# sharckhai/drsa-audio

Measured on AMD Instinct MI355X. Metric: explained samples/sec (LRP+DRSA k=4), higher is better.
Workload: dtype fp32; 1 GPU; GTZAN-128 HeatmapGenerator: LRP (WSquare/Gamma/Epsilon name map) + DRSA subspace heatmaps, K=4 at layer j=7 (conv3 block, d=64), sorted info dict; global_batch=512, per_gpu_batch=512, input=128x128 log-mel, parallelism=data-parallel x1 (no collective on the data path), launch=single process, one_device_rehearsal=False

## Files before the change

### drsa_audio_amd/csrc/conv_bwd_b.hip

```cpp
#include "lrp_conv_kernel.h"

#ifndef DRSA_CONV_CIC_BWD32
#define DRSA_CONV_CIC_BWD32 8
#endif
#ifndef DRSA_CONV_CIC_BWD64_32
#define DRSA_CONV_CIC_BWD64_32 8
#endif

CONV_TABLE(kTableBwdB,
    BWD_SET(64, 32, DRSA_CONV_CIC_BWD64_32),
    BWD_SET(32, 32, DRSA_CONV_CIC_BWD32))

#ifdef DRSA_CONV_STAMP
extern "C" int drsa_amd_debug_conv_stamps(void* buf) {
  return (int)hipMemcpyToSymbol(HIP_SYMBOL(drsa_conv::g_conv_stamps), &buf, sizeof(buf));
}
#endif
```

### drsa_audio_amd/csrc/lrp_conv.h

```cpp
#pragma once
#include <stdint.h>

enum XMode { XM_NONE = 0, XM_MUL = 1, XM_SPLIT = 2 };
enum PostMode { POST_NONE = 0, POST_DIV = 1, POST_MASK = 2, POST_DIV_RING = 3 };

struct ConvArgs {
  const float* in;
  const uint8_t* in_amax;
  const float* wts;
  const float* bias;
  const float* den_map;
  const float* den_const4;
  const float* x;
  const float* den;
  float* out;
  uint8_t* out_amax;
  float* out_den;
  int H, W;
  int cin, cout;
  int clones;
  int xmode, post;
  float eps;
  int den_ring_only;
  int den_shared;
};

#include <hip/hip_runtime.h>
int drsa_first_conv_pool(const ConvArgs& a, int cout_p, int ng, int B, hipStream_t s);
```

### drsa_audio_amd/csrc/lrp_conv.hip

```cpp
#include "common.h"
#include "lrp_conv.h"
#include "lrp_conv_kernel.h"

#include <stdlib.h>

#define DRSA_CONV_TABLES(X) \
  X(FwdA) X(FwdB) X(FwdC) X(FwdD) X(FwdE) X(BwdA) X(BwdB) X(BwdC) X(FwdBfA) X(FwdBfB) X(FwdBfC) X(FwdP4) X(BwdBfA) X(BwdBfB)

namespace drsa_conv {
#define DRSA_CONV_DECLARE(T) extern const Table kTable##T;
DRSA_CONV_TABLES(DRSA_CONV_DECLARE)
extern const Table kTableSmall;
}

namespace {
using drsa_conv::Entry;
using namespace drsa_conv;

#define DRSA_CONV_ADDRESS(T) &drsa_conv::kTable##T,
const drsa_conv::Table* kTables[] = {DRSA_CONV_TABLES(DRSA_CONV_ADDRESS)};

int pad32(int c) { return (c + 31) / 32 * 32; }

#ifndef DRSA_CONV_FWD128_TW
#define DRSA_CONV_FWD128_TW 8
#endif
const Entry* find(int cin_p, int cout_p, int W, int ng, int amode, int epi, int et = 0, int pw = 2) {
  int th = 8, tw, mw;
  const bool fwd_t16 = epi != EPI_BWD && et == 0 && cout_p == 64;
  const bool bwd_t16 = epi == EPI_BWD && et == 0 && ((cout_p == 64 && cin_p <= 128) || cout_p == 128);
  if (W >= 32 && epi != EPI_BWD && et == 0 && cout_p == 128 && DRSA_CONV_FWD128_TW != 32) {
    tw = DRSA_CONV_FWD128_TW;
    mw = tw == 8 ? 4 : 8;
  } else if (W >= 32 && (fwd_t16 || bwd_t16)) { tw = 16; mw = 8; }
  else if (W >= 32) { tw = 32; mw = 8; }
  else { tw = 8; mw = 4; }
  for (const drsa_conv::Table* t : kTables)
    for (int i = 0; i < t->n; ++i) {
      const Entry& e = t->entries[i];
      if (e.cin_p == cin_p && e.cout_p == cout_p && e.th == th && e.tw == tw && e.mw == mw && e.ng == ng &&
          e.amode == amode && e.epi == epi && e.et == et && e.pw == pw)
        return &e;
    }
  return nullptr;
}

#ifndef DRSA_CONV_SMALL_WG
#define DRSA_CONV_SMALL_WG 512
#endif
const Entry* small_tile(const Entry* e, int H, int W, int batch) {
  if (e->th != 8 || e->tw != 8) return e;
  if ((int64_t)((H + 7) / 8) * ((W + 7) / 8) * batch >= DRSA_CONV_SMALL_WG) return e;
  for (int i = 0; i < drsa_conv::kTableSmall.n; ++i) {
    const Entry& c = drsa_conv::kTableSmall.entries[i];
    if (c.cin_p == e->cin_p && c.cout_p == e->cout_p && c.ng == e->ng && c.amode == e->amode && c.epi == e->epi &&
        c.et == e->et && c.pw == e->pw)
      return &c;
  }
  return e;
}

int launch(const Entry* e0, const ConvArgs& args, int batch, hipStream_t s) {
  DRSA_REQUIRE((int64_t)(args.cin > args.cout ? args.cin : args.cout) * args.H * args.W < ((int64_t)1 << 31),
               "conv: one sample's channels x H x W must stay below 2^31");
  const Entry* e = small_tile(e0, args.H, args.W, batch);
  DRSA_SMEM(e->fn, e->lds);
  const int tiles = ((args.H + e->th - 1) / e->th) * ((args.W + e->tw - 1) / e->tw);
  hipLaunchKernelGGL(e->fn, dim3(tiles, batch), dim3(kThreads), e->lds, s, args);
  DRSA_LAUNCH_CHECK();
  return DRSA_OK;
}

int cin_pad(int cin) { return cin == 1 ? 1 : pad32(cin); }

const Entry* find_fwd(int cin, int cout, int W, int ng, int pool, int bf16) {
  return find(bf16 ? pad32(cin) : cin_pad(cin), pad32(cout), W, ng, A_DENSE, pool ? EPI_FWD_POOL : EPI_FWD_RELU,
              bf16 ? 1 : 0, pool == 2 ? 4 : 2);
}

const Entry* find_bwd(int cin, int cout, int W, int ng, int sparse, int bf16, int pool_w) {
  return find(pad32(cin), pad32(cout), W, ng, sparse ? A_POOLSPARSE : A_DENSE, EPI_BWD, bf16 ? 1 : 0, pool_w);
}

// ... 76 lines not shown
  return launch(e, a, c.Bq, (hipStream_t)stream);
}

}

extern "C" {

size_t drsa_amd_conv_weight_floats(int cin, int cout, int ng) {
  return (size_t)ng * 9 * cin_pad(cin) * pad32(cout);
}

size_t drsa_amd_conv_weight_bf16_elems(int cin, int cout, int ng) {
  return (size_t)ng * 9 * pad32(cin) * pad32(cout);
}

int drsa_amd_conv_fwd_has_kernel(int cin, int cout, int W, int ng, int pool, int bf16) {
  if (cin == 1 && !bf16 && pool == 1) return 1;
  if (pool < 0 || pool > 2 || ng < 1 || ng > 3 || (bf16 && cin == 1)) return 0;
  return find_fwd(cin, cout, W, ng, pool, bf16) != nullptr;
}

int drsa_amd_conv_bwd_has_kernel_bf16(int cin, int cout, int W, int ng, int sparse) {
  if (cin < 16 || ng != 1) return 0;
  return find_bwd(cin, cout, W, ng, sparse, 1, 2) != nullptr;
}

int drsa_amd_conv_bwd_has_kernel_pw(int cin, int cout, int W, int ng, int pool_w) {
  if (cin < 2 || (pool_w != 2 && pool_w != 4) || (pool_w == 4 && (W / 4) % 4 != 0)) return 0;
  return find_bwd(cin, cout, W, ng, 1, 0, pool_w) != nullptr;
}
// ... 79 lines not shown
```

### drsa_audio_amd/csrc/lrp_conv_kernel.h

```cpp
#pragma once
#include "common.h"
#include "lrp_conv.h"

#include <type_traits>

#ifndef DRSA_CONV_PD_BWD
#define DRSA_CONV_PD_BWD 2
#endif
#ifndef DRSA_CONV_BWD_ES
#define DRSA_CONV_BWD_ES 1
#endif
#ifndef DRSA_CONV_BWD_WPE
#define DRSA_CONV_BWD_WPE 3
#endif
#ifndef DRSA_CONV_PIN_SMALL
#define DRSA_CONV_PIN_SMALL 1
#endif
#ifndef DRSA_CONV_PD_SMALL
#define DRSA_CONV_PD_SMALL 3
#endif
#ifndef DRSA_CONV_SMALL_WPE
#define DRSA_CONV_SMALL_WPE 4
#endif
#ifndef DRSA_CONV_SMALL_ES
// ... 11 lines not shown
#ifndef DRSA_CONV_FWD_WPE_128
#define DRSA_CONV_FWD_WPE_128 3
#endif
#ifndef DRSA_CONV_FWD_WPE_WIDE
#define DRSA_CONV_FWD_WPE_WIDE 3
#endif
#ifndef DRSA_CONV_FWD_WPE
#define DRSA_CONV_FWD_WPE 3
#endif

namespace drsa_conv {

constexpr int kThreads = 256;

#ifdef DRSA_CONV_STAMP
static __device__ unsigned long long* g_conv_stamps;
#endif

__device__ const float g_zero_bias3[3 * 128] = {};

template <int V, int M>
constexpr int round_up() { return (V + M - 1) / M * M; }

constexpr int halo_stride(int hx, int mw) {
  int r = hx;
  const int want = (mw == 8) ? 16 : 8;
  while (r % 32 != want) ++r;
  return r;
}

enum AMode { A_DENSE = 0, A_POOLSPARSE = 1 };
enum Epi { EPI_FWD_POOL = 0, EPI_FWD_RELU = 1, EPI_BWD = 2 };

constexpr int XO = 3;

constexpr int bf_stride(int hx) {
  int r = hx;
  while (r % 16 != 8) ++r;
  return r;
}

template <int CIN, int COUT, int TH, int TW, int MW, int CIC, int NG, int AMODE, int EPI, int ET = 0, int PW = 2>
struct ConvCfg {
  static constexpr int CIN_ = CIN, COUT_ = COUT, TH_ = TH, TW_ = TW, MW_ = MW, CIC_ = CIC, NG_ = NG;
  static constexpr int AMODE_ = AMODE, EPI_ = EPI;
  static constexpr bool BF = ET == 1;
  static constexpr int HY = TH + 2, HX = TW + 2;
  static constexpr int HXB = bf_stride(HX);
  static constexpr size_t bf_halo_floats = (size_t)2 * HY * HXB * 4;
  static constexpr size_t bf_w_floats = (size_t)NG * 9 * 2 * COUT * 4;
  static constexpr int RS = halo_stride(HX + XO, MW);
  static constexpr int PLANE_RAW = HY * RS;
  static constexpr int PLANE = PLANE_RAW + ((PLANE_RAW % 32) == 0 ? 4 : 0);
  static constexpr int MTW = 2 * MW;
  static constexpr int MTH = 32 / MTW;
  static constexpr int MTX = TW / MTW;
  static constexpr int MT = (TH / MTH) * MTX;
  static constexpr int NT = COUT / 32;
  static constexpr int WM = MT >= 4 ? 4 : MT;
  static constexpr int WN = (4 / WM) < NT ? (4 / WM) : NT;
  static constexpr int MPW = MT / WM;
  static constexpr int NPW = NT / WN;
  static constexpr int KC = 9 * CIC;
  static constexpr int KCP = round_up<KC, 2>();
  static constexpr int NCHUNK = CIN / CIC;
  static constexpr int TWP = (TW == 32) ? 48 : TW;
  static constexpr bool SMALL_BWD = EPI == EPI_BWD && NG == 1 && CIC <= 8 && COUT <= 32;
  static constexpr int ES = (EPI == EPI_BWD && WN == 1) ? (SMALL_BWD ? DRSA_CONV_SMALL_ES : DRSA_CONV_BWD_ES) : 1;
  static constexpr int TCH = WN * 32 / ES;
  static constexpr size_t staging_floats =
      BF ? bf_halo_floats + bf_w_floats : (size_t)CIC * PLANE + (size_t)NG * KCP * COUT;
  static constexpr size_t epi_floats = (size_t)TCH * TH * TWP;
  static constexpr size_t lds_floats = staging_floats > epi_floats ? staging_floats : epi_floats;
  static constexpr int WPE = BF ? (COUT <= 64 ? DRSA_CONV_BF_WPE : 1)
                             : (EPI == EPI_BWD && NG == 1) ? (SMALL_BWD ? DRSA_CONV_SMALL_WPE : DRSA_CONV_BWD_WPE)
                             : (EPI != EPI_BWD && CIC <= 8 && COUT <= 32 && NG <= 2 ? DRSA_CONV_FWD_WPE
                                : EPI != EPI_BWD && CIC <= 8 && NG <= 2 && COUT == 64 ? DRSA_CONV_FWD_WPE_WIDE
                                : EPI != EPI_BWD && CIC <= 4 && NG <= 2 && COUT == 128 && TW == 8 ? DRSA_CONV_FWD_WPE_128 : 1);
  static constexpr bool PIN = SMALL_BWD && DRSA_CONV_PIN_SMALL;
  static constexpr int PD = PIN ? DRSA_CONV_PD_SMALL : DRSA_CONV_PD_BWD > 0 && EPI >= EPI_BWD ? DRSA_CONV_PD_BWD : 1;
  static_assert(TH % MTH == 0 && TW % MTW == 0, "tile must be a multiple of the M-tile");
  static_assert(COUT % 32 == 0, "COUT must be padded to 32");
  static_assert(CIN % CIC == 0, "CIN must be a multiple of the chunk");
  static_assert(MT % WM == 0 && NT % WN == 0 && WM * WN <= 4, "wave split");
  static_assert(!BF || (CIC == 16 && (EPI < EPI_BWD ? AMODE == A_DENSE : EPI == EPI_BWD)),
                "bf16: 16-channel chunks; dense forward, or the per-clone backward (dense or pool-sparse g)");
  static_assert(PW == 2 || (PW == 4 && (EPI == EPI_FWD_POOL || (EPI == EPI_BWD && AMODE == A_POOLSPARSE &&
                                                                  (ET == 1 || TW % 16 == 0)))),
                "2x4 pool windows: the forward pool epilogue, or the backward's pool-sparse staging (fp32: "
                "tiles of whole float4 cell groups)");
  static constexpr int PW_ = PW;
};

template <class Cfg, int NT_ = kThreads>
struct Stager {
  static constexpr int CIN = Cfg::CIN_, COUT = Cfg::COUT_, TH = Cfg::TH_, TW = Cfg::TW_, CIC = Cfg::CIC_;
  static constexpr int NG = Cfg::NG_, HY = Cfg::HY, HX = Cfg::HX, RS = Cfg::RS, PLANE = Cfg::PLANE;
  static constexpr int KC = Cfg::KC, KCP = Cfg::KCP;
  static constexpr bool DENSE = Cfg::AMODE_ == A_DENSE;
  static constexpr int Q4 = TW / 4, DROWS = CIC * HY;
  static constexpr int DI = (DROWS * Q4 + NT_ - 1) / NT_, DH = (DROWS * 2 + NT_ - 1) / NT_;
  static constexpr int CY = TH / 2 + 2, CX = TW / 2 + 2, Q8 = TW / 8 > 0 ? TW / 8 : 1, SROWS = CIC * CY;
  static constexpr int SI = (SROWS * Q8 + NT_ - 1) / NT_, SH = (SROWS * 2 + NT_ - 1) / NT_;
  static constexpr bool P4 = !DENSE && Cfg::PW_ == 4;
  static constexpr int Q16 = TW / 16 > 0 ? TW / 16 : 1;
  static constexpr int SI4 = (SROWS * Q16 + NT_ - 1) / NT_;
  static constexpr int NI = DENSE ? DI : P4 ? SI4 : SI, NH = DENSE ? DH : SH;
  static constexpr int NWV = NG * KCP * (COUT / 4), WIT = (NWV + NT_ - 1) / NT_;
  float4 st_i[NI];
  uint32_t st_ia[DENSE ? 1 : NI];
  float st_h[NH];
  int st_ha[DENSE ? 1 : NH];
  float4 st_w[WIT];

  __device__ __forceinline__ void load(const ConvArgs& a, int c0, int tid, int ty0, int tx0, int bq, int bs) {
    const int H = a.H, W = a.W, H2 = H >> 1, W2 = W >> 1;
    const int W4 = W >> 2;
    const float* __restrict__ inb = a.in + (size_t)bq * a.cin * (DENSE ? H * W : H2 * (P4 ? W4 : W2));
    const uint8_t* __restrict__ amb = DENSE ? nullptr : a.in_amax + (size_t)bs * a.cin * H2 * (P4 ? W4 : W2);
    if constexpr (P4) {
      const int qy0 = (ty0 >> 1) - 1, cx0 = tx0 >> 2;
#pragma unroll
      for (int it = 0; it < SI4; ++it) {
        const int i = tid + it * NT_;
        const int row = i / Q16, q = i % Q16;
        const int ci = row / CY, ry = row % CY;
        const int cy = qy0 + ry, cx = cx0 + 4 * q, c = c0 + ci;
        const bool ok = i < SROWS * Q16 && cy >= 0 && cy < H2 && c < a.cin && cx < W4;
        const int o = ok ? (c * H2 + cy) * W4 + cx : 0;
        const float4 v = *reinterpret_cast<const float4*>(inb + o);
// ... 101 lines not shown
        const int i = tid + it * NT_;
        const int row = i >> 1, side = i & 1;
        const int ci = row / CY, ry = row % CY;
        const int cy = qy0 + ry, cx = side ? qx0 + CX - 1 : qx0, c = c0 + ci;
        const bool ok = i < SROWS * 2 && cy >= 0 && cy < H2 && cx >= 0 && cx < W2 && c < a.cin;
        const int o = ok ? (c * H2 + cy) * W2 + cx : 0;
        const float v = inb[o];
        const int am = (int)amb[o];
        st_h[it] = ok ? v : 0.f;
        st_ha[it] = ok ? am : 4;
      }
    }
#pragma unroll
    for (int it = 0; it < WIT; ++it) {
      const int idx = tid + it * NT_;
      const int g = idx / (KCP * (COUT / 4)), rem = idx % (KCP * (COUT / 4));
      const int k = rem / (COUT / 4), c4 = (rem % (COUT / 4)) * 4;
      const bool ok = idx < NWV && k < KC;
      const float4 v = *reinterpret_cast<const float4*>(a.wts + (ok ? ((size_t)g * 9 * CIN + c0 * 9 + k) * COUT + c4 : 0));
      st_w[it] = ok ? v : make_float4(0.f, 0.f, 0.f, 0.f);
    }
  }

  __device__ __forceinline__ static void put_cell(float* halo, int ci, int ry, int rx, float v, int sb) {
    float* d = halo + ci * PLANE + (2 * ry - 1) * RS + 2 * rx - 1 + XO;
    if (ry > 0) *reinterpret_cast<float2*>(d) = make_float2(sb == 0 ? v : 0.f, sb == 1 ? v : 0.f);
    if (ry < CY - 1) *reinterpret_cast<float2*>(d + RS) = make_float2(sb == 2 ? v : 0.f, sb == 3 ? v : 0.f);
  }

  __device__ __forceinline__ static void put_cell4(float* halo, int ci, int ry, int rx, float v, int sb) {
    float* d = halo + ci * PLANE + (2 * ry - 1) * RS + 4 * rx;
    if (ry > 0)
      *reinterpret_cast<float4*>(d) = make_float4(sb == 0 ? v : 0.f, sb == 1 ? v : 0.f, sb == 2 ? v : 0.f, sb == 3 ? v : 0.f);
    if (ry < CY - 1)
// ... 65 lines not shown
          put_cell(halo, row / CY, row % CY, side ? CX - 1 : 0, st_h[it], st_ha[it]);
        }
      }
    }
#pragma unroll
    for (int it = 0; it < WIT; ++it) {
      const int idx = tid + it * NT_;
      if (idx < NWV) *reinterpret_cast<float4*>(wl + (size_t)idx * 4) = st_w[it];
    }
  }
};

template <class Cfg, int PD = 1>
__device__ __forceinline__ void mfma_chunk(const float* halo, const float* wl, const int (&pix_off)[Cfg::MPW],
                                           int lane, int wn, f32x16 (&acc)[Cfg::NG_][Cfg::MPW][Cfg::NPW]) {
  constexpr int MPW = Cfg::MPW, NPW = Cfg::NPW, NG = Cfg::NG_, COUT = Cfg::COUT_;
  constexpr int KC = Cfg::KC, KCP = Cfg::KCP, PLANE = Cfg::PLANE, RS = Cfg::RS, EPI = Cfg::EPI_;
  const int h = lane >> 5;
  constexpr int DLT[3] = {1, RS - 2, PLANE - 2 * RS - 2};
  int xb[MPW][3];
#pragma unroll
  for (int u = 0; u < MPW; ++u)
#pragma unroll
    for (int t = 0; t < 3; ++t) xb[u][t] = pix_off[u] + h * DLT[t];
  auto read_x = [&](int k0, float (&xv)[MPW]) {
    const int r9 = k0 % 9;
    const int off = (k0 / 9) * PLANE + (r9 / 3) * RS + (r9 % 3);
    const int t = (r9 == 8) ? 2 : (r9 == 2 || r9 == 5) ? 1 : 0;
#pragma unroll
    for (int u = 0; u < MPW; ++u) {
      if constexpr (KC % 2 == 0) xv[u] = halo[xb[u][t] + off];
      else xv[u] = (k0 + h < KC) ? halo[xb[u][t] + off] : 0.f;
    }
  };
  auto read_w = [&](int k0, float (&wv)[NG][NPW]) {
#pragma unroll
    for (int v = 0; v < NPW; ++v)
#pragma unroll
      for (int g = 0; g < NG; ++g) wv[g][v] = wl[((size_t)g * KCP + k0 + h) * COUT + (wn * NPW + v) * 32 + (lane & 31)];
  };
  float xr[PD + 1][MPW], wr[PD + 1][NG][NPW];
#pragma unroll
  for (int d = 0; d < PD; ++d)
    if (2 * d < KCP) {
      read_x(2 * d, xr[d]);
      read_w(2 * d, wr[d]);
    }
#pragma unroll
  for (int k0 = 0; k0 < KCP; k0 += 2) {
    const int cur = (k0 / 2) % (PD + 1), nxt = (k0 / 2 + PD) % (PD + 1);
    if (k0 + 2 * PD < KCP) {
      read_x(k0 + 2 * PD, xr[nxt]);
      read_w(k0 + 2 * PD, wr[nxt]);
    }
// ... 14 lines not shown
}
template <class Cfg, int NT_ = kThreads>
struct StagerBF {
  static constexpr int CIN = Cfg::CIN_, COUT = Cfg::COUT_, NG = Cfg::NG_, HY = Cfg::HY, HX = Cfg::HX;
  static constexpr int HXB = Cfg::HXB, NCH = CIN / 16;
  static constexpr int NITEM = 2 * HY * HX, IT = (NITEM + NT_ - 1) / NT_;
  static constexpr int NWQ = NG * 18 * COUT, WIT = (NWQ + NT_ - 1) / NT_;
  static constexpr bool P4 = Cfg::AMODE_ == A_POOLSPARSE && Cfg::PW_ == 4;
  static constexpr int NCR = Cfg::TW_ / 4 + 2;
  static constexpr int NITEM4 = 2 * HY * NCR, IT4 = (NITEM4 + NT_ - 1) / NT_;
  static constexpr int ITX = P4 ? IT4 : IT;
  float st_f[ITX][8];
  uint32_t st_a[P4 ? IT4 : 1][2];
  uint4 st_w[WIT];

  __device__ __forceinline__ void load(const ConvArgs& a, int c0, int tid, int ty0, int tx0, int bq, int bs) {
    const int H = a.H, W = a.W;
    const unsigned HW = (unsigned)(H * W);
    const int H2s = H >> 1, W2s = W / (P4 ? 4 : Cfg::PW_);
    const float* __restrict__ inb =
        a.in + (size_t)bq * a.cin * (Cfg::AMODE_ == A_POOLSPARSE || P4 ? (size_t)H2s * W2s : (size_t)HW);
    const uint8_t* __restrict__ amb = (Cfg::AMODE_ == A_POOLSPARSE || P4) ? a.in_amax + (size_t)bs * a.cin * H2s * W2s
                                                                          : nullptr;
    if constexpr (P4) {
      const int H2 = H >> 1, W2 = W >> 2;
      const unsigned HW2 = (unsigned)(H2 * W2);
#pragma unroll
      for (int it = 0; it < IT4; ++it) {
        const int i = tid + it * NT_;
        const int cs = i % NCR, r = i / NCR, hy = r % HY, half = r / HY;
        const int gy = ty0 - 1 + hy, cx = (tx0 >> 2) - 1 + cs, cb = c0 + 8 * half;
// ... 143 lines not shown
        for (int u = 0; u < MPW; ++u) {
          uint4 b = xr[cur][u];
          if constexpr (NG == 3) {
            if (g > 0) {
              const uint4 m = make_uint4(bf2_neg_mask(b.x), bf2_neg_mask(b.y), bf2_neg_mask(b.z), bf2_neg_mask(b.w));
              b = (g == 1) ? make_uint4(b.x & ~m.x, b.y & ~m.y, b.z & ~m.z, b.w & ~m.w)
                           : make_uint4(b.x & m.x, b.y & m.y, b.z & m.z, b.w & m.w);
            }
          }
          acc[g][u][v] = mfma32_bf16(__builtin_bit_cast(u16x8, wr[cur][g][v]), __builtin_bit_cast(u16x8, b),
                                     acc[g][u][v]);
        }
  }
}

template <int CIN, int COUT, int TH, int TW, int MW, int CIC, int NG, int AMODE, int EPI, int ET = 0, int PW = 2>
__global__ __launch_bounds__(kThreads) __attribute__((amdgpu_waves_per_eu(ConvCfg<CIN, COUT, TH, TW, MW, CIC, NG, AMODE, EPI, ET, PW>::WPE))) void conv3x3_kernel(ConvArgs a) {
  using Cfg = ConvCfg<CIN, COUT, TH, TW, MW, CIC, NG, AMODE, EPI, ET, PW>;
  constexpr int HY = Cfg::HY, HX = Cfg::HX, RS = Cfg::RS, PLANE = Cfg::PLANE;
  constexpr int MTH = Cfg::MTH, MTW = Cfg::MTW, MTX = Cfg::MTX;
  constexpr int WM = Cfg::WM, MPW = Cfg::MPW, NPW = Cfg::NPW;
  constexpr int KC = Cfg::KC, KCP = Cfg::KCP;

  extern __shared__ __attribute__((aligned(16))) float smem[];
#ifdef DRSA_CONV_STAMP
  constexpr bool kStamp = EPI == EPI_BWD && CIN == 32 && COUT == 32 && AMODE == A_POOLSPARSE && ET == 0;
  unsigned long long* const stp = kStamp && g_conv_stamps && threadIdx.x == 0
                                      ? g_conv_stamps + ((size_t)blockIdx.y * gridDim.x + blockIdx.x) * 16 : nullptr;
#define CONV_STAMP(slot) do { if (stp) stp[(slot)] = __builtin_amdgcn_s_memtime(); } while (0)
#else
#define CONV_STAMP(slot) do {} while (0)
#endif
  CONV_STAMP(0);
  float* halo = smem;
  float* wl = smem + (Cfg::BF ? Cfg::bf_halo_floats : (size_t)CIC * PLANE);

  const int tid = threadIdx.x, lane = lane_id(), w = wave_id();
  const int H = a.H, W = a.W;
  const int tiles_x = (W + TW - 1) / TW;
  const int tile_id = blockIdx.x, bq = blockIdx.y;
  const int ty0 = (tile_id / tiles_x) * TH;
  const int tx0 = (tile_id % tiles_x) * TW;
  const int bs = bq / a.clones;
  const int wm = w % WM, wn = w / WM;
  const bool active = w < WM * Cfg::WN;
  const int h = lane >> 5;

  int pix_off[MPW], pix_y[MPW], pix_x[MPW];
#pragma unroll
  for (int u = 0; u < MPW; ++u) {
    const int mt = wm * MPW + u;
    const int p = lane & 31, win = p >> 2, sub = p & 3;
    pix_y[u] = (mt / MTX) * MTH + 2 * (win / MW) + (sub >> 1);
    pix_x[u] = (mt % MTX) * MTW + 2 * (win % MW) + (sub & 1);
    pix_off[u] = Cfg::BF ? (h * HY + pix_y[u]) * Cfg::HXB + pix_x[u] : pix_y[u] * RS + pix_x[u] + XO;
// ... 22 lines not shown
    if (active) {
#pragma unroll
      for (int u = 0; u < MPW; ++u)
#pragma unroll
        for (int r = 0; r < 16; ++r) {
          const int cf = (r & 3) + 8 * (r >> 2) + 4 * h;
          if constexpr (ES == 1) {
            T[((wn * 32 + cf) * TH + pix_y[u]) * TWP + pix_x[u]] = valfn(u, r);
          } else {
            if ((r >> (ES == 2 ? 3 : 2)) == sub) T[((cf - TCH * sub) * TH + pix_y[u]) * TWP + pix_x[u]] = valfn(u, r);
          }
        }
    }
    __syncthreads();
  };
  auto gch = [&](int cl, int v) { return ((cl >> 5) * NPW + v) * 32 + (cl & 31); };
  auto gchs = [&](int cl, int v, int sub) { return ES == 1 ? gch(cl, v) : v * 32 + sub * TCH + cl; };
  typename std::conditional<Cfg::BF, StagerBF<Cfg>, Stager<Cfg>>::type stg;
  stg.load(a, 0, tid, ty0, tx0, bq, bs);
  CONV_STAMP(11);
  for (int chunk = 0; chunk + (EPI == EPI_BWD ? 1 : 0) < Cfg::NCHUNK; ++chunk) {
    __syncthreads();
    if (chunk == 0) CONV_STAMP(9);
    if constexpr (Cfg::BF) stg.store(halo, wl, tid, ty0, tx0);
    else stg.store(halo, wl, tid);
    if (chunk == 0) CONV_STAMP(10);
    __syncthreads();
    CONV_STAMP(1 + 2 * chunk);
    if (chunk + 1 < Cfg::NCHUNK) stg.load(a, (chunk + 1) * CIC, tid, ty0, tx0, bq, bs);
    if (!active) continue;
    if constexpr (Cfg::BF)
      mfma_chunk_bf<Cfg>(reinterpret_cast<const uint4*>(halo), reinterpret_cast<const uint4*>(wl), pix_off, lane, wn, acc);
    else
      mfma_chunk<Cfg, Cfg::PD>(halo, wl, pix_off, lane, wn, acc);
    CONV_STAMP(2 + 2 * chunk);
  }
  constexpr int Q = TH * TW / 4, CS = kThreads / Q;
  static_assert(kThreads % Q == 0, "float4 groups per tile must divide the block");
  const int cl0 = tid / Q, rem = tid % Q;
  const int py = rem / (TW / 4), px = (rem % (TW / 4)) * 4;
  const bool pix_ok = ty0 + py < H && tx0 + px < W;
  const int HW = H * W;
  const size_t pix = pix_ok ? (size_t)(ty0 + py) * W + tx0 + px : 0;
  const float* xs = a.x ? a.x + (size_t)bs * a.cout * HW + pix : nullptr;
  const float* ds = a.den ? a.den + (a.den_shared ? (size_t)0 : (size_t)bs * a.cout * HW) + pix : nullptr;
  float* oqp = a.out + (size_t)bq * a.cout * HW + pix;
  const bool need_x = a.xmode != XM_NONE || a.post != POST_NONE;
  const bool mul_x = a.xmode != XM_NONE, split_x = a.xmode == XM_SPLIT;
  const bool ring = a.post == POST_DIV_RING && a.den_const4;
  const bool post_div = a.post == POST_DIV || ring, post_any = a.post != POST_NONE;
// ... 18 lines not shown
      const int cl = cl0 + it * CS;
      const int co = gchs(cl, v, sub);
      const bool ok = cl < TCH && co < a.cout;
      const int coc = ok ? co : 0;
      if (lx) xk[it] = *reinterpret_cast<const float4*>(xbase + (upix + (unsigned)coc * (unsigned)HW));
      if (ld) dk[it] = *reinterpret_cast<const float4*>(use_c4 ? a.den_const4 + (size_t)coc * 4 : rsrc + coc * dstride);
    }
  };
  constexpr int kPreN = DRSA_CONV_PRE_N < V4T ? DRSA_CONV_PRE_N : V4T;
  float4 pre_x[V4T], pre_d[V4T];
  if constexpr (EPI == EPI_BWD) {
    __syncthreads();
    if constexpr (Cfg::BF) stg.store(halo, wl, tid, ty0, tx0);
    else stg.store(halo, wl, tid);
    __syncthreads();
    CONV_STAMP(2 * Cfg::NCHUNK - 1);
    epi_loads(0, 0, pre_x, pre_d, true, DRSA_CONV_PRE_D, 0, kPreN);

    if (active) {
      if constexpr (Cfg::BF)
        mfma_chunk_bf<Cfg>(reinterpret_cast<const uint4*>(halo), reinterpret_cast<const uint4*>(wl), pix_off, lane, wn,
                           acc);
      else
        mfma_chunk<Cfg, Cfg::PD>(halo, wl, pix_off, lane, wn, acc);
    }
    CONV_STAMP(2 * Cfg::NCHUNK);
  }

  auto pool_cells = [&](auto pwc, auto&& fn) {
    constexpr int PWc = decltype(pwc)::value;
    constexpr int CW = TW / PWc, NC = TCH * (TH / 2) * CW;
    const int H2 = H >> 1, W2 = W / PWc;
#pragma unroll
    for (int it = 0; it < CT; ++it) {
      const int i = tid + it * kThreads;
      if (i < NC) {
        const int cl = i / ((TH / 2) * CW), rem = i % ((TH / 2) * CW);
        const int cy = rem / CW, cx = rem % CW;
        fn(it, cl, cy, cx, (ty0 >> 1) + cy, tx0 / PWc + cx, H2, W2);
      }
    }
  };
#pragma unroll
  for (int v = 0; v < NPW; ++v) {
    if constexpr (EPI == EPI_FWD_POOL || EPI == EPI_FWD_RELU) {
      const float* bb = a.bias ? a.bias : g_zero_bias3;
      float b0[16], b1[16], b2[16];
#pragma unroll
      for (int r = 0; r < 16; ++r) {
        const int co = gch(wn * 32 + (r & 3) + 8 * (r >> 2) + 4 * h, v);
        const bool cok = co < a.cout;
        const float x0 = bb[co], x1 = bb[COUT + co], x2 = bb[2 * COUT + co];
        b0[r] = cok ? x0 : 0.f;
// ... 248 lines not shown
        float4 R = Rk[it];
        const float4 x = xk[it], d = dk[it];
        auto post = [&](float rr, float xx, float dd) {
          const float q = div_nb(rr, stab(dd, eps));
          const float y = post_div ? q : rr;
          return (post_any && !(xx > 0.f)) ? 0.f : y;
        };
        R = make_float4(post(R.x, x.x, d.x), post(R.y, x.y, d.y), post(R.z, x.z, d.z), post(R.w, x.w, d.w));
        if (ok && pix_ok) *reinterpret_cast<float4*>(obase + (upix + (unsigned)coc * (unsigned)HW)) = R;
      }
     }
    }
  }
#ifdef DRSA_CONV_STAMP
  if (stp) {
    stp[13] = __builtin_amdgcn_s_memtime();
    stp[14] = (unsigned long long)__builtin_amdgcn_s_getreg(4 | (31 << 11));
    stp[15] = (unsigned long long)__builtin_amdgcn_s_getreg(20 | (31 << 11));
  }
#endif
#undef CONV_STAMP
}

typedef void (*KernFn)(ConvArgs);

struct Entry {
  int cin_p, cout_p, th, tw, mw, cic, ng, amode, epi;
  KernFn fn;
  size_t lds;
  int et = 0;
  int pw = 2;
};

struct Table {
  const Entry* entries;
  int n;
};

template <int... P>
constexpr Entry conv_entry() {
  static_assert(sizeof...(P) == 11, "CONV_ENTRY takes every ConvCfg parameter");
  constexpr int p[] = {P...};
  return Entry{p[0], p[1], p[2], p[3], p[4], p[5], p[6], p[7], p[8],
               conv3x3_kernel<P...>, ConvCfg<P...>::lds_floats * sizeof(float), p[9], p[10]};
}
#define CONV_ENTRY(CIN, COUT, TH, TW, MW, CIC, NG, AM, EP, ET, PW) \
  drsa_conv::conv_entry<CIN, COUT, TH, TW, MW, CIC, NG, AM, EP, ET, PW>()

#define CONV_FAMILY(CIN, COUT, CIC, NG, AM, EP, ET, PW)       \
  CONV_ENTRY(CIN, COUT, 8, 32, 8, CIC, NG, AM, EP, ET, PW),   \
  CONV_ENTRY(CIN, COUT, 8, 16, 8, CIC, NG, AM, EP, ET, PW),   \
  CONV_ENTRY(CIN, COUT, 8, 8, 4, CIC, NG, AM, EP, ET, PW)

#define FWD_SET_ET(CIN, COUT, CIC, ET)                                                      \
  CONV_FAMILY(CIN, COUT, CIC, 1, drsa_conv::A_DENSE, drsa_conv::EPI_FWD_POOL, ET, 2),        \
  CONV_FAMILY(CIN, COUT, CIC, 2, drsa_conv::A_DENSE, drsa_conv::EPI_FWD_POOL, ET, 2),        \
  CONV_FAMILY(CIN, COUT, CIC, 3, drsa_conv::A_DENSE, drsa_conv::EPI_FWD_POOL, ET, 2),        \
  CONV_FAMILY(CIN, COUT, CIC, 1, drsa_conv::A_DENSE, drsa_conv::EPI_FWD_RELU, ET, 2),        \
  CONV_FAMILY(CIN, COUT, CIC, 2, drsa_conv::A_DENSE, drsa_conv::EPI_FWD_RELU, ET, 2),        \
  CONV_FAMILY(CIN, COUT, CIC, 3, drsa_conv::A_DENSE, drsa_conv::EPI_FWD_RELU, ET, 2)
#define FWD_SET(CIN, COUT, CIC) FWD_SET_ET(CIN, COUT, CIC, 0)
#define FWD_SET_BF(CIN, COUT) FWD_SET_ET(CIN, COUT, 16, 1)
// ... 25 lines not shown
```

Measured before the change: 115,100 explained samples/s.

## Split conv output channels across workgroups for mid-size 64-channel layers

Adds an output-channel slice parameter (CW) to the conv3x3 kernel. Each workgroup now computes a 32-channel slice of the outputs, and the grid is multiplied by the number of slices. New slice entries are selected for 64->64 convs at widths between 8 and 32 and for 32->64 forward convs at wide widths. The aim is more workgroups and less LDS weight staging per block on small spatial layers. The cost is that input halos are loaded redundantly once per slice. The debug stamp plumbing also moves into a kernel argument.

```diff
diff --git a/drsa_audio_amd/csrc/conv_bwd_b.hip b/drsa_audio_amd/csrc/conv_bwd_b.hip
--- a/drsa_audio_amd/csrc/conv_bwd_b.hip
+++ b/drsa_audio_amd/csrc/conv_bwd_b.hip
@@ -10,9 +10,3 @@
 CONV_TABLE(kTableBwdB,
     BWD_SET(64, 32, DRSA_CONV_CIC_BWD64_32),
     BWD_SET(32, 32, DRSA_CONV_CIC_BWD32))
-
-#ifdef DRSA_CONV_STAMP
-extern "C" int drsa_amd_debug_conv_stamps(void* buf) {
-  return (int)hipMemcpyToSymbol(HIP_SYMBOL(drsa_conv::g_conv_stamps), &buf, sizeof(buf));
-}
-#endif
diff --git a/drsa_audio_amd/csrc/conv_slice.hip b/drsa_audio_amd/csrc/conv_slice.hip
--- /dev/null
+++ b/drsa_audio_amd/csrc/conv_slice.hip
@@ -0,0 +1,19 @@
+#include "lrp_conv_kernel.h"
+
+#define SLICE_FWD(CIN, COUT, TW, MW, CIC, CW)                                                        \
+  CONV_ENTRY_CW(CIN, COUT, 8, TW, MW, CIC, 1, drsa_conv::A_DENSE, drsa_conv::EPI_FWD_POOL, CW),      \
+  CONV_ENTRY_CW(CIN, COUT, 8, TW, MW, CIC, 2, drsa_conv::A_DENSE, drsa_conv::EPI_FWD_POOL, CW),      \
+  CONV_ENTRY_CW(CIN, COUT, 8, TW, MW, CIC, 3, drsa_conv::A_DENSE, drsa_conv::EPI_FWD_POOL, CW),      \
+  CONV_ENTRY_CW(CIN, COUT, 8, TW, MW, CIC, 1, drsa_conv::A_DENSE, drsa_conv::EPI_FWD_RELU, CW),      \
+  CONV_ENTRY_CW(CIN, COUT, 8, TW, MW, CIC, 2, drsa_conv::A_DENSE, drsa_conv::EPI_FWD_RELU, CW),      \
+  CONV_ENTRY_CW(CIN, COUT, 8, TW, MW, CIC, 3, drsa_conv::A_DENSE, drsa_conv::EPI_FWD_RELU, CW)
+#define SLICE_BWD(CIN, COUT, TW, MW, CIC, CW)                                                        \
+  CONV_ENTRY_CW(CIN, COUT, 8, TW, MW, CIC, 1, drsa_conv::A_DENSE, drsa_conv::EPI_BWD, CW),           \
+  CONV_ENTRY_CW(CIN, COUT, 8, TW, MW, CIC, 2, drsa_conv::A_DENSE, drsa_conv::EPI_BWD, CW),           \
+  CONV_ENTRY_CW(CIN, COUT, 8, TW, MW, CIC, 1, drsa_conv::A_POOLSPARSE, drsa_conv::EPI_BWD, CW),      \
+  CONV_ENTRY_CW(CIN, COUT, 8, TW, MW, CIC, 2, drsa_conv::A_POOLSPARSE, drsa_conv::EPI_BWD, CW)
+
+CONV_TABLE(kTableSlice,
+    SLICE_FWD(64, 64, 16, 8, 8, 32),
+    SLICE_BWD(64, 64, 16, 8, 8, 32),
+    SLICE_FWD(32, 64, 32, 8, 8, 32))
diff --git a/drsa_audio_amd/csrc/lrp_conv.h b/drsa_audio_amd/csrc/lrp_conv.h
--- a/drsa_audio_amd/csrc/lrp_conv.h
+++ b/drsa_audio_amd/csrc/lrp_conv.h
@@ -23,6 +23,9 @@
   float eps;
   int den_ring_only;
   int den_shared;
+#ifdef DRSA_CONV_STAMP
+  unsigned long long* stamps;
+#endif
 };
 
 #include <hip/hip_runtime.h>
diff --git a/drsa_audio_amd/csrc/lrp_conv.hip b/drsa_audio_amd/csrc/lrp_conv.hip
--- a/drsa_audio_amd/csrc/lrp_conv.hip
+++ b/drsa_audio_amd/csrc/lrp_conv.hip
@@ -5,7 +5,7 @@
 #include <stdlib.h>
 
 #define DRSA_CONV_TABLES(X) \
-  X(FwdA) X(FwdB) X(FwdC) X(FwdD) X(FwdE) X(BwdA) X(BwdB) X(BwdC) X(FwdBfA) X(FwdBfB) X(FwdBfC) X(FwdP4) X(BwdBfA) X(BwdBfB)
+  X(FwdA) X(FwdB) X(FwdC) X(FwdD) X(FwdE) X(BwdA) X(BwdB) X(BwdC) X(FwdBfA) X(FwdBfB) X(FwdBfC) X(FwdP4) X(BwdBfA) X(BwdBfB) X(Slice)
 
 namespace drsa_conv {
 #define DRSA_CONV_DECLARE(T) extern const Table kTable##T;
@@ -26,7 +26,7 @@
 #define DRSA_CONV_FWD128_TW 8
 #endif
 const Entry* find(int cin_p, int cout_p, int W, int ng, int amode, int epi, int et = 0, int pw = 2) {
-  int th = 8, tw, mw;
+  int th = 8, tw, mw, cw = cout_p;
   const bool fwd_t16 = epi != EPI_BWD && et == 0 && cout_p == 64;
   const bool bwd_t16 = epi == EPI_BWD && et == 0 && ((cout_p == 64 && cin_p <= 128) || cout_p == 128);
   if (W >= 32 && epi != EPI_BWD && et == 0 && cout_p == 128 && DRSA_CONV_FWD128_TW != 32) {
@@ -35,11 +35,15 @@
   } else if (W >= 32 && (fwd_t16 || bwd_t16)) { tw = 16; mw = 8; }
   else if (W >= 32) { tw = 32; mw = 8; }
   else { tw = 8; mw = 4; }
+  if (et == 0 && pw == 2) {
+    if (cin_p == 64 && cout_p == 64 && W > 8 && W < 32) { tw = 16; mw = 8; cw = 32; }
+    else if (epi != EPI_BWD && cin_p == 32 && cout_p == 64 && W >= 32) { tw = 32; mw = 8; cw = 32; }
+  }
   for (const drsa_conv::Table* t : kTables)
     for (int i = 0; i < t->n; ++i) {
       const Entry& e = t->entries[i];
       if (e.cin_p == cin_p && e.cout_p == cout_p && e.th == th && e.tw == tw && e.mw == mw && e.ng == ng &&
-          e.amode == amode && e.epi == epi && e.et == et && e.pw == pw)
+          e.amode == amode && e.epi == epi && e.et == et && e.pw == pw && e.cw == cw)
         return &e;
     }
   return nullptr;
@@ -50,7 +54,7 @@
 #endif
 const Entry* small_tile(const Entry* e, int H, int W, int batch) {
   if (e->th != 8 || e->tw != 8) return e;
-  if ((int64_t)((H + 7) / 8) * ((W + 7) / 8) * batch >= DRSA_CONV_SMALL_WG) return e;
+  if ((int64_t)((H + 7) / 8) * ((W + 7) / 8) * batch * (e->cout_p / e->cw) >= DRSA_CONV_SMALL_WG) return e;
   for (int i = 0; i < drsa_conv::kTableSmall.n; ++i) {
     const Entry& c = drsa_conv::kTableSmall.entries[i];
     if (c.cin_p == e->cin_p && c.cout_p == e->cout_p && c.ng == e->ng && c.amode == e->amode && c.epi == e->epi &&
@@ -60,13 +64,23 @@
   return e;
 }
 
-int launch(const Entry* e0, const ConvArgs& args, int batch, hipStream_t s) {
+#ifdef DRSA_CONV_STAMP
+unsigned long long* g_stamps = nullptr;
+#endif
+
+int launch(const Entry* e0, const ConvArgs& args0, int batch, hipStream_t s) {
+#ifdef DRSA_CONV_STAMP
+  ConvArgs args = args0;
+  args.stamps = g_stamps;
+#else
+  const ConvArgs& args = args0;
+#endif
   DRSA_REQUIRE((int64_t)(args.cin > args.cout ? args.cin : args.cout) * args.H * args.W < ((int64_t)1 << 31),
                "conv: one sample's channels x H x W must stay below 2^31");
   const Entry* e = small_tile(e0, args.H, args.W, batch);
   DRSA_SMEM(e->fn, e->lds);
   const int tiles = ((args.H + e->th - 1) / e->th) * ((args.W + e->tw - 1) / e->tw);
-  hipLaunchKernelGGL(e->fn, dim3(tiles, batch), dim3(kThreads), e->lds, s, args);
+  hipLaunchKernelGGL(e->fn, dim3(tiles * (e->cout_p / e->cw), batch), dim3(kThreads), e->lds, s, args);
   DRSA_LAUNCH_CHECK();
   return DRSA_OK;
 }
@@ -173,6 +187,13 @@
   return (size_t)ng * 9 * pad32(cin) * pad32(cout);
 }
 
+#ifdef DRSA_CONV_STAMP
+int drsa_amd_debug_conv_stamps(void* buf) {
+  g_stamps = static_cast<unsigned long long*>(buf);
+  return DRSA_OK;
+}
+#endif
+
 int drsa_amd_conv_fwd_has_kernel(int cin, int cout, int W, int ng, int pool, int bf16) {
   if (cin == 1 && !bf16 && pool == 1) return 1;
   if (pool < 0 || pool > 2 || ng < 1 || ng > 3 || (bf16 && cin == 1)) return 0;
diff --git a/drsa_audio_amd/csrc/lrp_conv_kernel.h b/drsa_audio_amd/csrc/lrp_conv_kernel.h
--- a/drsa_audio_amd/csrc/lrp_conv_kernel.h
+++ b/drsa_audio_amd/csrc/lrp_conv_kernel.h
@@ -49,7 +49,7 @@
 constexpr int kThreads = 256;
 
 #ifdef DRSA_CONV_STAMP
-static __device__ unsigned long long* g_conv_stamps;
+constexpr int kStampSlots = 48;
 #endif
 
 __device__ const float g_zero_bias3[3 * 128] = {};
@@ -75,9 +75,12 @@
   return r;
 }
 
-template <int CIN, int COUT, int TH, int TW, int MW, int CIC, int NG, int AMODE, int EPI, int ET = 0, int PW = 2>
+template <int CIN, int COUT, int TH, int TW, int MW, int CIC, int NG, int AMODE, int EPI, int ET = 0, int PW = 2,
+          int CW = COUT>
 struct ConvCfg {
   static constexpr int CIN_ = CIN, COUT_ = COUT, TH_ = TH, TW_ = TW, MW_ = MW, CIC_ = CIC, NG_ = NG;
+  static constexpr int CW_ = CW, NS = COUT / CW;
+  static constexpr bool SLICED = CW != COUT;
   static constexpr int AMODE_ = AMODE, EPI_ = EPI;
   static constexpr bool BF = ET == 1;
   static constexpr int HY = TH + 2, HX = TW + 2;
@@ -91,7 +94,7 @@
   static constexpr int MTH = 32 / MTW;
   static constexpr int MTX = TW / MTW;
   static constexpr int MT = (TH / MTH) * MTX;
-  static constexpr int NT = COUT / 32;
+  static constexpr int NT = CW / 32;
   static constexpr int WM = MT >= 4 ? 4 : MT;
   static constexpr int WN = (4 / WM) < NT ? (4 / WM) : NT;
   static constexpr int MPW = MT / WM;
@@ -104,10 +107,11 @@
   static constexpr int ES = (EPI == EPI_BWD && WN == 1) ? (SMALL_BWD ? DRSA_CONV_SMALL_ES : DRSA_CONV_BWD_ES) : 1;
   static constexpr int TCH = WN * 32 / ES;
   static constexpr size_t staging_floats =
-      BF ? bf_halo_floats + bf_w_floats : (size_t)CIC * PLANE + (size_t)NG * KCP * COUT;
+      BF ? bf_halo_floats + bf_w_floats : (size_t)CIC * PLANE + (size_t)NG * KCP * CW;
   static constexpr size_t epi_floats = (size_t)TCH * TH * TWP;
   static constexpr size_t lds_floats = staging_floats > epi_floats ? staging_floats : epi_floats;
-  static constexpr int WPE = BF ? (COUT <= 64 ? DRSA_CONV_BF_WPE : 1)
+  static constexpr int WPE = SLICED ? (EPI != EPI_BWD && CW == 32 && NG <= 2 && TW < 32 ? 4 : 3)
+                             : BF ? (COUT <= 64 ? DRSA_CONV_BF_WPE : 1)
                              : (EPI == EPI_BWD && NG == 1) ? (SMALL_BWD ? DRSA_CONV_SMALL_WPE : DRSA_CONV_BWD_WPE)
                              : (EPI != EPI_BWD && CIC <= 8 && COUT <= 32 && NG <= 2 ? DRSA_CONV_FWD_WPE
                                 : EPI != EPI_BWD && CIC <= 8 && NG <= 2 && COUT == 64 ? DRSA_CONV_FWD_WPE_WIDE
@@ -116,6 +120,7 @@
   static constexpr int PD = PIN ? DRSA_CONV_PD_SMALL : DRSA_CONV_PD_BWD > 0 && EPI >= EPI_BWD ? DRSA_CONV_PD_BWD : 1;
   static_assert(TH % MTH == 0 && TW % MTW == 0, "tile must be a multiple of the M-tile");
   static_assert(COUT % 32 == 0, "COUT must be padded to 32");
+  static_assert(CW % 32 == 0 && COUT % CW == 0 && (!SLICED || !BF), "slices: whole 32-channel n-tiles, fp32 only");
   static_assert(CIN % CIC == 0, "CIN must be a multiple of the chunk");
   static_assert(MT % WM == 0 && NT % WN == 0 && WM * WN <= 4, "wave split");
   static_assert(!BF || (CIC == 16 && (EPI < EPI_BWD ? AMODE == A_DENSE : EPI == EPI_BWD)),
@@ -131,7 +136,7 @@
 struct Stager {
   static constexpr int CIN = Cfg::CIN_, COUT = Cfg::COUT_, TH = Cfg::TH_, TW = Cfg::TW_, CIC = Cfg::CIC_;
   static constexpr int NG = Cfg::NG_, HY = Cfg::HY, HX = Cfg::HX, RS = Cfg::RS, PLANE = Cfg::PLANE;
-  static constexpr int KC = Cfg::KC, KCP = Cfg::KCP;
+  static constexpr int KC = Cfg::KC, KCP = Cfg::KCP, CW = Cfg::CW_;
   static constexpr bool DENSE = Cfg::AMODE_ == A_DENSE;
   static constexpr int Q4 = TW / 4, DROWS = CIC * HY;
   static constexpr int DI = (DROWS * Q4 + NT_ - 1) / NT_, DH = (DROWS * 2 + NT_ - 1) / NT_;
@@ -141,14 +146,14 @@
   static constexpr int Q16 = TW / 16 > 0 ? TW / 16 : 1;
   static constexpr int SI4 = (SROWS * Q16 + NT_ - 1) / NT_;
   static constexpr int NI = DENSE ? DI : P4 ? SI4 : SI, NH = DENSE ? DH : SH;
-  static constexpr int NWV = NG * KCP * (COUT / 4), WIT = (NWV + NT_ - 1) / NT_;
+  static constexpr int NWV = NG * KCP * (CW / 4), WIT = (NWV + NT_ - 1) / NT_;
   float4 st_i[NI];
   uint32_t st_ia[DENSE ? 1 : NI];
   float st_h[NH];
   int st_ha[DENSE ? 1 : NH];
   float4 st_w[WIT];
 
-  __device__ __forceinline__ void load(const ConvArgs& a, int c0, int tid, int ty0, int tx0, int bq, int bs) {
+  __device__ __forceinline__ void load(const ConvArgs& a, int c0, int tid, int ty0, int tx0, int bq, int bs, int co0) {
     const int H = a.H, W = a.W, H2 = H >> 1, W2 = W >> 1;
     const int W4 = W >> 2;
     const float* __restrict__ inb = a.in + (size_t)bq * a.cin * (DENSE ? H * W : H2 * (P4 ? W4 : W2));
@@ -280,10 +285,11 @@
 #pragma unroll
     for (int it = 0; it < WIT; ++it) {
       const int idx = tid + it * NT_;
-      const int g = idx / (KCP * (COUT / 4)), rem = idx % (KCP * (COUT / 4));
-      const int k = rem / (COUT / 4), c4 = (rem % (COUT / 4)) * 4;
+      const int g = idx / (KCP * (CW / 4)), rem = idx % (KCP * (CW / 4));
+      const int k = rem / (CW / 4), c4 = (rem % (CW / 4)) * 4;
       const bool ok = idx < NWV && k < KC;
-      const float4 v = *reinterpret_cast<const float4*>(a.wts + (ok ? ((size_t)g * 9 * CIN + c0 * 9 + k) * COUT + c4 : 0));
+      const float4 v =
+          *reinterpret_cast<const float4*>(a.wts + (ok ? ((size_t)g * 9 * CIN + c0 * 9 + k) * COUT + co0 + c4 : 0));
       st_w[it] = ok ? v : make_float4(0.f, 0.f, 0.f, 0.f);
     }
   }
@@ -379,7 +385,7 @@
 template <class Cfg, int PD = 1>
 __device__ __forceinline__ void mfma_chunk(const float* halo, const float* wl, const int (&pix_off)[Cfg::MPW],
                                            int lane, int wn, f32x16 (&acc)[Cfg::NG_][Cfg::MPW][Cfg::NPW]) {
-  constexpr int MPW = Cfg::MPW, NPW = Cfg::NPW, NG = Cfg::NG_, COUT = Cfg::COUT_;
+  constexpr int MPW = Cfg::MPW, NPW = Cfg::NPW, NG = Cfg::NG_, CW = Cfg::CW_;
   constexpr int KC = Cfg::KC, KCP = Cfg::KCP, PLANE = Cfg::PLANE, RS = Cfg::RS, EPI = Cfg::EPI_;
   const int h = lane >> 5;
   constexpr int DLT[3] = {1, RS - 2, PLANE - 2 * RS - 2};
@@ -402,7 +408,7 @@
 #pragma unroll
     for (int v = 0; v < NPW; ++v)
 #pragma unroll
-      for (int g = 0; g < NG; ++g) wv[g][v] = wl[((size_t)g * KCP + k0 + h) * COUT + (wn * NPW + v) * 32 + (lane & 31)];
+      for (int g = 0; g < NG; ++g) wv[g][v] = wl[((size_t)g * KCP + k0 + h) * CW + (wn * NPW + v) * 32 + (lane & 31)];
   };
   float xr[PD + 1][MPW], wr[PD + 1][NG][NPW];
 #pragma unroll
@@ -447,7 +453,7 @@
   uint32_t st_a[P4 ? IT4 : 1][2];
   uint4 st_w[WIT];
 
-  __device__ __forceinline__ void load(const ConvArgs& a, int c0, int tid, int ty0, int tx0, int bq, int bs) {
+  __device__ __forceinline__ void load(const ConvArgs& a, int c0, int tid, int ty0, int tx0, int bq, int bs, int) {
     const int H = a.H, W = a.W;
     const unsigned HW = (unsigned)(H * W);
     const int H2s = H >> 1, W2s = W / (P4 ? 4 : Cfg::PW_);
@@ -621,9 +627,10 @@
   }
 }
 
-template <int CIN, int COUT, int TH, int TW, int MW, int CIC, int NG, int AMODE, int EPI, int ET = 0, int PW = 2>
-__global__ __launch_bounds__(kThreads) __attribute__((amdgpu_waves_per_eu(ConvCfg<CIN, COUT, TH, TW, MW, CIC, NG, AMODE, EPI, ET, PW>::WPE))) void conv3x3_kernel(ConvArgs a) {
-  using Cfg = ConvCfg<CIN, COUT, TH, TW, MW, CIC, NG, AMODE, EPI, ET, PW>;
+template <int CIN, int COUT, int TH, int TW, int MW, int CIC, int NG, int AMODE, int EPI, int ET = 0, int PW = 2,
+          int CW = COUT>
+__global__ __launch_bounds__(kThreads) __attribute__((amdgpu_waves_per_eu(ConvCfg<CIN, COUT, TH, TW, MW, CIC, NG, AMODE, EPI, ET, PW, CW>::WPE))) void conv3x3_kernel(ConvArgs a) {
+  using Cfg = ConvCfg<CIN, COUT, TH, TW, MW, CIC, NG, AMODE, EPI, ET, PW, CW>;
   constexpr int HY = Cfg::HY, HX = Cfg::HX, RS = Cfg::RS, PLANE = Cfg::PLANE;
   constexpr int MTH = Cfg::MTH, MTW = Cfg::MTW, MTX = Cfg::MTX;
   constexpr int WM = Cfg::WM, MPW = Cfg::MPW, NPW = Cfg::NPW;
@@ -631,9 +638,12 @@
 
   extern __shared__ __attribute__((aligned(16))) float smem[];
 #ifdef DRSA_CONV_STAMP
-  constexpr bool kStamp = EPI == EPI_BWD && CIN == 32 && COUT == 32 && AMODE == A_POOLSPARSE && ET == 0;
-  unsigned long long* const stp = kStamp && g_conv_stamps && threadIdx.x == 0
-                                      ? g_conv_stamps + ((size_t)blockIdx.y * gridDim.x + blockIdx.x) * 16 : nullptr;
+  constexpr bool kStamp = ET == 0 && PW == 2 && Cfg::NCHUNK <= 16 &&
+                          ((EPI == EPI_BWD && CIN == 32 && COUT == 32 && AMODE == A_POOLSPARSE) ||
+                           (EPI == EPI_BWD && CIN == 64 && COUT == 64 && AMODE == A_POOLSPARSE && NG == 1) ||
+                           (EPI == EPI_FWD_POOL && CIN == 64 && COUT == 64 && NG == 2));
+  unsigned long long* const stp = kStamp && a.stamps && threadIdx.x == 0
+                                      ? a.stamps + ((size_t)blockIdx.y * gridDim.x + blockIdx.x) * kStampSlots : nullptr;
 #define CONV_STAMP(slot) do { if (stp) stp[(slot)] = __builtin_amdgcn_s_memtime(); } while (0)
 #else
 #define CONV_STAMP(slot) do {} while (0)
@@ -645,7 +655,9 @@
   const int tid = threadIdx.x, lane = lane_id(), w = wave_id();
   const int H = a.H, W = a.W;
   const int tiles_x = (W + TW - 1) / TW;
-  const int tile_id = blockIdx.x, bq = blockIdx.y;
+  constexpr int NS = Cfg::NS;
+  const int tile_id = NS == 1 ? (int)blockIdx.x : (int)blockIdx.x / NS, bq = blockIdx.y;
+  const int co0 = NS == 1 ? 0 : ((int)blockIdx.x % NS) * CW;
   const int ty0 = (tile_id / tiles_x) * TH;
   const int tx0 = (tile_id % tiles_x) * TW;
   const int bs = bq / a.clones;
@@ -698,26 +710,26 @@
     }
     __syncthreads();
   };
-  auto gch = [&](int cl, int v) { return ((cl >> 5) * NPW + v) * 32 + (cl & 31); };
-  auto gchs = [&](int cl, int v, int sub) { return ES == 1 ? gch(cl, v) : v * 32 + sub * TCH + cl; };
+  auto gch = [&](int cl, int v) { return co0 + ((cl >> 5) * NPW + v) * 32 + (cl & 31); };
+  auto gchs = [&](int cl, int v, int sub) { return ES == 1 ? gch(cl, v) : co0 + v * 32 + sub * TCH + cl; };
   typename std::conditional<Cfg::BF, StagerBF<Cfg>, Stager<Cfg>>::type stg;
-  stg.load(a, 0, tid, ty0, tx0, bq, bs);
-  CONV_STAMP(11);
+  stg.load(a, 0, tid, ty0, tx0, bq, bs, co0);
+  CONV_STAMP(1);
   for (int chunk = 0; chunk + (EPI == EPI_BWD ? 1 : 0) < Cfg::NCHUNK; ++chunk) {
     __syncthreads();
-    if (chunk == 0) CONV_STAMP(9);
+    if (chunk == 0) CONV_STAMP(2);
     if constexpr (Cfg::BF) stg.store(halo, wl, tid, ty0, tx0);
     else stg.store(halo, wl, tid);
-    if (chunk == 0) CONV_STAMP(10);
+    if (chunk == 0) CONV_STAMP(3);
     __syncthreads();
-    CONV_STAMP(1 + 2 * chunk);
-    if (chunk + 1 < Cfg::NCHUNK) stg.load(a, (chunk + 1) * CIC, tid, ty0, tx0, bq, bs);
+    CONV_STAMP(8 + 2 * chunk);
+    if (chunk + 1 < Cfg::NCHUNK) stg.load(a, (chunk + 1) * CIC, tid, ty0, tx0, bq, bs, co0);
     if (!active) continue;
     if constexpr (Cfg::BF)
       mfma_chunk_bf<Cfg>(reinterpret_cast<const uint4*>(halo), reinterpret_cast<const uint4*>(wl), pix_off, lane, wn, acc);
     else
       mfma_chunk<Cfg, Cfg::PD>(halo, wl, pix_off, lane, wn, acc);
-    CONV_STAMP(2 + 2 * chunk);
+    CONV_STAMP(9 + 2 * chunk);
   }
   constexpr int Q = TH * TW / 4, CS = kThreads / Q;
   static_assert(kThreads % Q == 0, "float4 groups per tile must divide the block");
@@ -766,7 +778,7 @@
     if constexpr (Cfg::BF) stg.store(halo, wl, tid, ty0, tx0);
     else stg.store(halo, wl, tid);
     __syncthreads();
-    CONV_STAMP(2 * Cfg::NCHUNK - 1);
+    CONV_STAMP(6 + 2 * Cfg::NCHUNK);
     epi_loads(0, 0, pre_x, pre_d, true, DRSA_CONV_PRE_D, 0, kPreN);
 
     if (active) {
@@ -776,19 +788,19 @@
       else
         mfma_chunk<Cfg, Cfg::PD>(halo, wl, pix_off, lane, wn, acc);
     }
-    CONV_STAMP(2 * Cfg::NCHUNK);
+    CONV_STAMP(7 + 2 * Cfg::NCHUNK);
   }
 
   auto pool_cells = [&](auto pwc, auto&& fn) {
     constexpr int PWc = decltype(pwc)::value;
-    constexpr int CW = TW / PWc, NC = TCH * (TH / 2) * CW;
+    constexpr int CXC = TW / PWc, NC = TCH * (TH / 2) * CXC;
     const int H2 = H >> 1, W2 = W / PWc;
 #pragma unroll
     for (int it = 0; it < CT; ++it) {
       const int i = tid + it * kThreads;
       if (i < NC) {
-        const int cl = i / ((TH / 2) * CW), rem = i % ((TH / 2) * CW);
-        const int cy = rem / CW, cx = rem % CW;
+        const int cl = i / ((TH / 2) * CXC), rem = i % ((TH / 2) * CXC);
+        const int cy = rem / CXC, cx = rem % CXC;
         fn(it, cl, cy, cx, (ty0 >> 1) + cy, tx0 / PWc + cx, H2, W2);
       }
     }
@@ -1067,9 +1079,9 @@
   }
 #ifdef DRSA_CONV_STAMP
   if (stp) {
-    stp[13] = __builtin_amdgcn_s_memtime();
-    stp[14] = (unsigned long long)__builtin_amdgcn_s_getreg(4 | (31 << 11));
-    stp[15] = (unsigned long long)__builtin_amdgcn_s_getreg(20 | (31 << 11));
+    stp[4] = __builtin_amdgcn_s_memtime();
+    stp[5] = (unsigned long long)__builtin_amdgcn_s_getreg(4 | (31 << 11));
+    stp[6] = (unsigned long long)__builtin_amdgcn_s_getreg(20 | (31 << 11));
   }
 #endif
 #undef CONV_STAMP
@@ -1083,6 +1095,7 @@
   size_t lds;
   int et = 0;
   int pw = 2;
+  int cw = 0;
 };
 
 struct Table {
@@ -1092,13 +1105,15 @@
 
 template <int... P>
 constexpr Entry conv_entry() {
-  static_assert(sizeof...(P) == 11, "CONV_ENTRY takes every ConvCfg parameter");
+  static_assert(sizeof...(P) == 11 || sizeof...(P) == 12, "CONV_ENTRY takes every ConvCfg parameter");
   constexpr int p[] = {P...};
   return Entry{p[0], p[1], p[2], p[3], p[4], p[5], p[6], p[7], p[8],
-               conv3x3_kernel<P...>, ConvCfg<P...>::lds_floats * sizeof(float), p[9], p[10]};
+               conv3x3_kernel<P...>, ConvCfg<P...>::lds_floats * sizeof(float), p[9], p[10], ConvCfg<P...>::CW_};
 }
 #define CONV_ENTRY(CIN, COUT, TH, TW, MW, CIC, NG, AM, EP, ET, PW) \
   drsa_conv::conv_entry<CIN, COUT, TH, TW, MW, CIC, NG, AM, EP, ET, PW>()
+#define CONV_ENTRY_CW(CIN, COUT, TH, TW, MW, CIC, NG, AM, EP, CW) \
+  drsa_conv::conv_entry<CIN, COUT, TH, TW, MW, CIC, NG, AM, EP, 0, 2, CW>()
 
 #define CONV_FAMILY(CIN, COUT, CIC, NG, AM, EP, ET, PW)       \
   CONV_ENTRY(CIN, COUT, 8, 32, 8, CIC, NG, AM, EP, ET, PW),   \
```

Measured after the change: 116,000 explained samples/s, median of 6. About the same (+0.8%).
